# microsoft/tf-gnn-samples

Measured on AMD Instinct MI355X. Metric: edges/sec (whole node), RGCN PPI h=256 training, distinct batches (the reference's epoch-loop definition), higher is better.
Workload: dtype f32; 1 GPU; C2: RGCN on synthetic PPI-shaped batches (~16 graphs, ~1.88 M edges, ~32 k nodes each), 3 edge types [fwd,self,bkwd], h=256, 3 layers, sum aggregation, 1/in-de…; graphs_per_rank=64, max_nodes_in_batch=35964, input_pipeline=ResidentDataset, parallelism=dp1-by-graph

## Files before the change

### tf_gnn_samples_amd/csrc/seg_reduce.hip

```cpp
#include "common.h"

#include <stdlib.h>

using namespace relgnn;

namespace {

constexpr int kUnroll = 8;

__device__ __forceinline__ float act_apply(int act, float x) {
  switch (act) {
    case RELGNN_ACT_TANH: return act_fwd<RELGNN_ACT_TANH>(x);
    case RELGNN_ACT_RELU: return act_fwd<RELGNN_ACT_RELU>(x);
    case RELGNN_ACT_LEAKY_RELU: return act_fwd<RELGNN_ACT_LEAKY_RELU>(x);
    case RELGNN_ACT_ELU: return act_fwd<RELGNN_ACT_ELU>(x);
    case RELGNN_ACT_SELU: return act_fwd<RELGNN_ACT_SELU>(x);
    case RELGNN_ACT_GELU: return act_fwd<RELGNN_ACT_GELU>(x);
    default: return x;
  }
}

__device__ __forceinline__ float msg_act_apply(int act, float x) {
  switch (act) {
    case RELGNN_ACT_TANH: return act_fwd_fast<RELGNN_ACT_TANH>(x);
    case RELGNN_ACT_RELU: return act_fwd_fast<RELGNN_ACT_RELU>(x);
    case RELGNN_ACT_LEAKY_RELU: return act_fwd_fast<RELGNN_ACT_LEAKY_RELU>(x);
    case RELGNN_ACT_ELU: return act_fwd_fast<RELGNN_ACT_ELU>(x);
    case RELGNN_ACT_SELU: return act_fwd_fast<RELGNN_ACT_SELU>(x);
    case RELGNN_ACT_GELU: return act_fwd_fast<RELGNN_ACT_GELU>(x);
    default: return x;
  }
}

__device__ __forceinline__ uint32_t wave_max_u32(uint32_t v) {
  v = max(v, (uint32_t)__builtin_amdgcn_update_dpp(0, (int)v, 0xB1, 0xF, 0xF, true));
  v = max(v, (uint32_t)__builtin_amdgcn_update_dpp(0, (int)v, 0x4E, 0xF, 0xF, true));
  v = max(v, (uint32_t)__builtin_amdgcn_update_dpp(0, (int)v, 0x141, 0xF, 0xF, true));
  v = max(v, (uint32_t)__builtin_amdgcn_update_dpp(0, (int)v, 0x140, 0xF, 0xF, true));
  v = max(v, (uint32_t)__builtin_amdgcn_update_dpp(0, (int)v, 0x142, 0xA, 0xF, true));
  v = max(v, (uint32_t)__builtin_amdgcn_update_dpp(0, (int)v, 0x143, 0xC, 0xF, true));
  return (uint32_t)__builtin_amdgcn_readlane((int)v, 63);
}

template <bool IS_MAX, bool MSGACT = false>
__device__ __forceinline__ void combine(float4& acc, float w, const float4& v, int msg_act = RELGNN_ACT_LINEAR) {
  float4 m = make_float4(w * v.x, w * v.y, w * v.z, w * v.w);
  if constexpr (MSGACT) {
    m.x = msg_act_apply(msg_act, m.x); m.y = msg_act_apply(msg_act, m.y);
    m.z = msg_act_apply(msg_act, m.z); m.w = msg_act_apply(msg_act, m.w);
  }
  if constexpr (IS_MAX) {
    acc.x = fmaxf(acc.x, m.x); acc.y = fmaxf(acc.y, m.y);
    acc.z = fmaxf(acc.z, m.z); acc.w = fmaxf(acc.w, m.w);
  } else {
    acc.x += m.x; acc.y += m.y; acc.z += m.z; acc.w += m.w;
  }
}

__device__ __forceinline__ void combine64(double (&acc)[4], float w, const float4& v) {
  const double wd = (double)w;
  acc[0] = fma(wd, (double)v.x, acc[0]); acc[1] = fma(wd, (double)v.y, acc[1]);
  acc[2] = fma(wd, (double)v.z, acc[2]); acc[3] = fma(wd, (double)v.w, acc[3]);
}

__device__ __forceinline__ float4 finalize(int mode, int act, float4 a, int n) {
  if (mode == RELGNN_AGG_MEAN) {
    float d = (float)max(n, 1);
    a.x /= d; a.y /= d; a.z /= d; a.w /= d;
  } else if (mode == RELGNN_AGG_SQRT_N) {
    float d = sqrtf((float)max(n, 1));
    a.x /= d; a.y /= d; a.z /= d; a.w /= d;
  }
  if (act != RELGNN_ACT_LINEAR) {
    a.x = act_apply(act, a.x); a.y = act_apply(act, a.y);
    a.z = act_apply(act, a.z); a.w = act_apply(act, a.w);
  }
  return a;
}

template <int NCH, bool IS_MAX, bool HAS_W, int UNROLL = kUnroll, bool NT = false, bool XCD = true, bool MSGACT = false,
          bool ACC64 = false>
__global__ __launch_bounds__(256) void seg_reduce_wave_kernel(
    const float4* __restrict__ X, int64_t ldx4, int32_t D4, const int32_t* __restrict__ rowptr,
    int64_t num_segments, int32_t stride, const int32_t* __restrict__ col,
    const float* __restrict__ w, int32_t mode, int32_t act, float4* __restrict__ out, int64_t ldo4,
    int64_t n_logical_blocks, int32_t col_block0, int32_t msg_act, float* __restrict__ rowmax) {
  const int64_t lb = XCD ? xcd_logical_block(n_logical_blocks)
                         : ((int64_t)blockIdx.x < n_logical_blocks ? (int64_t)blockIdx.x : -1);
  if (lb < 0) return;
  const int lane = threadIdx.x & 63;
  const int64_t s = lb * 4 + (threadIdx.x >> 6);
  if (s >= num_segments) return;

  const int beg = __builtin_amdgcn_readfirstlane(rowptr[s * stride]);
  const int end = __builtin_amdgcn_readfirstlane(rowptr[(s + 1) * stride]);

  const int c0 = (col_block0 + (int)blockIdx.y * NCH) * 64 + lane;
  static_assert(!ACC64 || (!IS_MAX && !MSGACT), "float64 accumulation: plain sums only");
  float4 acc[NCH];
  double accd[ACC64 ? NCH : 1][4];
  bool on[NCH];
  uint32_t cc[NCH];
#pragma unroll
  for (int c = 0; c < NCH; ++c) {
    const float init = IS_MAX ? -FLT_MAX : 0.f;
    acc[c] = make_float4(init, init, init, init);
    if constexpr (ACC64) accd[c][0] = accd[c][1] = accd[c][2] = accd[c][3] = 0.0;
    on[c] = (c0 + 64 * c) < D4;
    cc[c] = (uint32_t)min(c0 + 64 * c, D4 - 1);
  }
  const uint32_t ld = (uint32_t)ldx4;

  for (int p = beg; p < end; p += 64) {
    const int n = min(64, end - p);
    const int my_col = (lane < n) ? (NT ? __builtin_nontemporal_load(col + p + lane) : col[p + lane]) : 0;
    float my_w = 1.f;
    if constexpr (HAS_W) my_w = (lane < n) ? (NT ? __builtin_nontemporal_load(w + p + lane) : w[p + lane]) : 0.f;

    int k = 0;
    for (; k + UNROLL <= n; k += UNROLL) {
      float4 v[UNROLL][NCH];
      float ww[UNROLL];
#pragma unroll
      for (int u = 0; u < UNROLL; ++u) {
        const uint32_t r = (uint32_t)__builtin_amdgcn_readlane(my_col, k + u);
        ww[u] = HAS_W ? __int_as_float(__builtin_amdgcn_readlane(__float_as_int(my_w), k + u)) : 1.f;
        const float4* row = X + (size_t)(r * ld);
#pragma unroll
        for (int c = 0; c < NCH; ++c) v[u][c] = row[cc[c]];
      }
#pragma unroll
      for (int u = 0; u < UNROLL; ++u)
#pragma unroll
        for (int c = 0; c < NCH; ++c) {
          if constexpr (ACC64) combine64(accd[c], ww[u], v[u][c]);
          else combine<IS_MAX, MSGACT>(acc[c], ww[u], v[u][c], msg_act);
        }
    }
    for (; k < n; ++k) {
      const uint32_t r = (uint32_t)__builtin_amdgcn_readlane(my_col, k);
      const float wk = HAS_W ? __int_as_float(__builtin_amdgcn_readlane(__float_as_int(my_w), k)) : 1.f;
      const float4* row = X + (size_t)(r * ld);
#pragma unroll
      for (int c = 0; c < NCH; ++c) {
        float4 v = row[cc[c]];
        if constexpr (ACC64) combine64(accd[c], wk, v);
        else combine<IS_MAX, MSGACT>(acc[c], wk, v, msg_act);
      }
    }
  }
  if constexpr (ACC64) {
#pragma unroll
    for (int c = 0; c < NCH; ++c)
      acc[c] = make_float4((float)accd[c][0], (float)accd[c][1], (float)accd[c][2], (float)accd[c][3]);
  }

  float4* orow = out + s * ldo4 + c0;
  uint32_t mxb = 0u, mxf = 0u;
  auto absb = [](float x) { return __float_as_uint(x) & 0x7FFFFFFFu; };
  auto finb = [](float x) { const uint32_t u = __float_as_uint(x) & 0x7FFFFFFFu; return u < 0x7F800000u ? u : 0u; };
#pragma unroll
  for (int c = 0; c < NCH; ++c)
    if (on[c]) {
      const float4 r = finalize(mode, act, acc[c], end - beg);
      mxb = max(max(mxb, max(absb(r.x), absb(r.y))), max(absb(r.z), absb(r.w)));
      if (__builtin_expect(mxb >= 0x7F800000u, 0))
        mxf = max(max(mxf, max(finb(r.x), finb(r.y))), max(finb(r.z), finb(r.w)));
      else
        mxf = mxb;
      if constexpr (NT) {
        float* o = reinterpret_cast<float*>(orow + 64 * c);
        __builtin_nontemporal_store(r.x, o); __builtin_nontemporal_store(r.y, o + 1);
        __builtin_nontemporal_store(r.z, o + 2); __builtin_nontemporal_store(r.w, o + 3);
      } else {
        orow[64 * c] = r;
      }
    }
  if (rowmax) {
    const uint32_t m = wave_max_u32(mxf);
    if (lane == 0) rowmax[s] = __uint_as_float(m);
  }
}

template <int GROUP, bool IS_MAX, bool HAS_W, bool MSGACT = false>
__global__ __launch_bounds__(256) void seg_reduce_group_kernel(
    const float4* __restrict__ X, int64_t ldx4, int32_t D4, const int32_t* __restrict__ rowptr,
    int64_t num_segments, int32_t stride, const int32_t* __restrict__ col,
    const float* __restrict__ w, int32_t mode, int32_t act, float4* __restrict__ out, int64_t ldo4,
    int64_t n_logical_blocks, int32_t msg_act) {
  constexpr int SEGS_PER_WAVE = 64 / GROUP;
  constexpr int U = 4;
  const int64_t lb = xcd_logical_block(n_logical_blocks);
  if (lb < 0) return;
  const int lane = threadIdx.x & 63;
  const int g = lane / GROUP, gl = lane % GROUP;
  const int64_t s = (lb * 4 + (threadIdx.x >> 6)) * SEGS_PER_WAVE + g;
  const bool valid = s < num_segments;
  const int beg = valid ? rowptr[s * stride] : 0;
  const int end = valid ? rowptr[(s + 1) * stride] : 0;
  const int len = end - beg;
  int maxlen = len;
#pragma unroll
  for (int off = 32; off >= GROUP; off >>= 1) maxlen = max(maxlen, __shfl_xor(maxlen, off));
  maxlen = __builtin_amdgcn_readfirstlane(maxlen);

  const bool on = gl < D4;
  const float init = IS_MAX ? -FLT_MAX : 0.f;
  float4 acc = make_float4(init, init, init, init);
  const float4* Xl = X + min(gl, D4 - 1);
  const uint32_t ld = (uint32_t)ldx4;

  for (int p0 = 0; p0 < maxlen; p0 += GROUP) {
    const int idx = p0 + gl;
    const int my_col = (idx < len) ? col[beg + idx] : 0;
    float my_w = 1.f;
    if constexpr (HAS_W) my_w = (idx < len) ? w[beg + idx] : 0.f;
    const int nn = min(GROUP, maxlen - p0);
    for (int k = 0; k < nn; k += U) {
      float4 v[U];
      float ww[U];
#pragma unroll
      for (int u = 0; u < U; ++u) {
        const uint32_t r = (uint32_t)__shfl(my_col, (k + u) & (GROUP - 1), GROUP);
        ww[u] = HAS_W ? __shfl(my_w, (k + u) & (GROUP - 1), GROUP) : 1.f;
        v[u] = Xl[(size_t)(r * ld)];
      }
#pragma unroll
      for (int u = 0; u < U; ++u) {
        float4 t = acc;
        combine<IS_MAX, MSGACT>(t, ww[u], v[u], msg_act);
        if (p0 + k + u < len) acc = t;
      }
    }
  }
  if (valid && on) out[s * ldo4 + gl] = finalize(mode, act, acc, len);
}

template <bool IS_MAX>
__global__ __launch_bounds__(256) void seg_reduce_scalar_kernel(
    const float* __restrict__ X, int64_t ldx, int32_t D, const int32_t* __restrict__ rowptr,
    int64_t num_segments, int32_t stride, const int32_t* __restrict__ col,
    const float* __restrict__ w, int32_t mode, int32_t act, float* __restrict__ out, int64_t ldo, int32_t msg_act) {
  const int lane = threadIdx.x & 63;
  const int64_t s = (int64_t)blockIdx.x * 4 + (threadIdx.x >> 6);
  if (s >= num_segments) return;
  const int beg = rowptr[s * stride], end = rowptr[(s + 1) * stride];
  for (int d = lane; d < D; d += 64) {
    float acc = IS_MAX ? -FLT_MAX : 0.f;
    for (int p = beg; p < end; ++p) {
      float m = msg_act_apply(msg_act, (w ? w[p] : 1.f) * X[(int64_t)col[p] * ldx + d]);
      acc = IS_MAX ? fmaxf(acc, m) : acc + m;
    }
    float nrm = (float)max(end - beg, 1);
    if (mode == RELGNN_AGG_MEAN) acc /= nrm;
    if (mode == RELGNN_AGG_SQRT_N) acc /= sqrtf(nrm);
    out[s * ldo + d] = act_apply(act, acc);
  }
}

__global__ __launch_bounds__(256) void seg_max_count_kernel(
    const float* __restrict__ X, int64_t ldx, int32_t D, const int32_t* __restrict__ rowptr,
    int64_t num_segments, int32_t stride, const int32_t* __restrict__ col,
    const float* __restrict__ w, const float* __restrict__ out, const float* __restrict__ gout,
    int64_t ldo, float* __restrict__ gsel) {
  const int lane = threadIdx.x & 63;
  const int64_t s = (int64_t)blockIdx.x * 4 + (threadIdx.x >> 6);
  if (s >= num_segments) return;
  const int beg = rowptr[s * stride], end = rowptr[(s + 1) * stride];
  for (int d = lane; d < D; d += 64) {
    const float o = out[s * ldo + d];
    float cnt = 0.f;
    for (int p = beg; p < end; ++p) {
      float m = (w ? w[p] : 1.f) * X[(int64_t)col[p] * ldx + d];
      cnt += (m == o) ? 1.f : 0.f;
    }
    gsel[s * ldo + d] = cnt > 0.f ? gout[s * ldo + d] / cnt : 0.f;
  }
}

__global__ __launch_bounds__(256) void seg_max_bwd_kernel(
    const float* __restrict__ X, int64_t ldx, int32_t D, const int32_t* __restrict__ rowptr_b,
    int64_t num_rows, int32_t stride_b, const int32_t* __restrict__ seg_b,
    const float* __restrict__ w_b, const float* __restrict__ out, const float* __restrict__ gsel,
    int64_t ldo, float* __restrict__ gX, int64_t ldgx) {
  const int lane = threadIdx.x & 63;
  const int64_t r = (int64_t)blockIdx.x * 4 + (threadIdx.x >> 6);
  if (r >= num_rows) return;
  const int beg = rowptr_b[r * stride_b], end = rowptr_b[(r + 1) * stride_b];
  for (int d = lane; d < D; d += 64) {
    const float x = X[r * ldx + d];
    float acc = 0.f;
    for (int q = beg; q < end; ++q) {
      const float wq = w_b ? w_b[q] : 1.f;
      const int64_t s = seg_b[q];
      if (wq * x == out[s * ldo + d]) acc += wq * gsel[s * ldo + d];
    }
    gX[r * ldgx + d] = acc;
  }
}

__device__ __forceinline__ float4 eq4(float4 a, float4 b) {
  return make_float4(a.x == b.x ? 1.f : 0.f, a.y == b.y ? 1.f : 0.f, a.z == b.z ? 1.f : 0.f, a.w == b.w ? 1.f : 0.f);
}

template <int G>
__global__ __launch_bounds__(256) void seg_max_count_vec_kernel(
    const float4* __restrict__ X, int64_t ldx4, int32_t D4, const int32_t* __restrict__ rowptr, int64_t num_segments,
    int32_t stride, const int32_t* __restrict__ col, const float* __restrict__ w, const float4* __restrict__ out,
    const float4* __restrict__ gout, int64_t ldo4, float4* __restrict__ gsel, int64_t nlb) {
  constexpr int U = 4;
  const int64_t lb = xcd_logical_block(nlb);
  if (lb < 0) return;
  const int lane = threadIdx.x & 63, g = lane / G, gl = lane % G;
  const int64_t s = (lb * 4 + (threadIdx.x >> 6)) * (64 / G) + g;
  if (s >= num_segments) return;
  const int beg = rowptr[s * stride], end = rowptr[(s + 1) * stride];
  for (int c = gl; c < D4; c += G) {
    const float4 o = out[s * ldo4 + c];
    float4 cnt = make_float4(0.f, 0.f, 0.f, 0.f);
    for (int p = beg; p < end; p += U) {
      int r[U];
      float ww[U];
      float4 v[U];
#pragma unroll
      for (int u = 0; u < U; ++u) {
        const int idx = min(p + u, end - 1);
        r[u] = col[idx];
        ww[u] = w ? w[idx] : 1.f;
      }
#pragma unroll
      for (int u = 0; u < U; ++u) v[u] = X[(int64_t)r[u] * ldx4 + c];
#pragma unroll
      for (int u = 0; u < U; ++u)
        if (p + u < end) {
          const float4 e = eq4(make_float4(ww[u] * v[u].x, ww[u] * v[u].y, ww[u] * v[u].z, ww[u] * v[u].w), o);
          cnt.x += e.x; cnt.y += e.y; cnt.z += e.z; cnt.w += e.w;
        }
    }
    const float4 gg = gout[s * ldo4 + c];
    gsel[s * ldo4 + c] = make_float4(cnt.x > 0.f ? gg.x / cnt.x : 0.f, cnt.y > 0.f ? gg.y / cnt.y : 0.f,
                                     cnt.z > 0.f ? gg.z / cnt.z : 0.f, cnt.w > 0.f ? gg.w / cnt.w : 0.f);
  }
}

template <int G>
__global__ __launch_bounds__(256) void seg_max_bwd_vec_kernel(
    const float4* __restrict__ X, int64_t ldx4, int32_t D4, const int32_t* __restrict__ rowptr_b, int64_t num_rows,
    int32_t stride_b, const int32_t* __restrict__ seg_b, const float* __restrict__ w_b, const float4* __restrict__ out,
    const float4* __restrict__ gsel, int64_t ldo4, float4* __restrict__ gX, int64_t ldgx4, int64_t nlb) {
  constexpr int U = 4;
  const int64_t lb = xcd_logical_block(nlb);
  if (lb < 0) return;
  const int lane = threadIdx.x & 63, g = lane / G, gl = lane % G;
  const int64_t r = (lb * 4 + (threadIdx.x >> 6)) * (64 / G) + g;
  if (r >= num_rows) return;
  const int beg = rowptr_b[r * stride_b], end = rowptr_b[(r + 1) * stride_b];
  for (int c = gl; c < D4; c += G) {
    const float4 x = X[r * ldx4 + c];
    float4 acc = make_float4(0.f, 0.f, 0.f, 0.f);
    for (int q = beg; q < end; q += U) {
      int sg[U];
      float wq[U];
      float4 o[U], gs[U];
#pragma unroll
      for (int u = 0; u < U; ++u) {
        const int idx = min(q + u, end - 1);
        sg[u] = seg_b[idx];
        wq[u] = w_b ? w_b[idx] : 1.f;
      }
#pragma unroll
      for (int u = 0; u < U; ++u) {
        o[u] = out[(int64_t)sg[u] * ldo4 + c];
        gs[u] = gsel[(int64_t)sg[u] * ldo4 + c];
      }
#pragma unroll
      for (int u = 0; u < U; ++u)
        if (q + u < end) {
          const float4 e = eq4(make_float4(wq[u] * x.x, wq[u] * x.y, wq[u] * x.z, wq[u] * x.w), o[u]);
          acc.x += e.x != 0.f ? wq[u] * gs[u].x : 0.f; acc.y += e.y != 0.f ? wq[u] * gs[u].y : 0.f;
          acc.z += e.z != 0.f ? wq[u] * gs[u].z : 0.f; acc.w += e.w != 0.f ? wq[u] * gs[u].w : 0.f;
        }
    }
    gX[r * ldgx4 + c] = acc;
  }
}

template <int ACT>
__global__ __launch_bounds__(256) void act_bwd_from_output_kernel(const float* __restrict__ y,
                                                                  const float* __restrict__ gout,
                                                                  int64_t n, float* __restrict__ gin) {
  for (int64_t i = blockIdx.x * (int64_t)blockDim.x + threadIdx.x; i < n;
       i += (int64_t)gridDim.x * blockDim.x) {
    const float yy = y[i], g = gout[i];
    float d = 1.f;
    if constexpr (ACT == RELGNN_ACT_TANH) d = 1.f - yy * yy;
    if constexpr (ACT == RELGNN_ACT_RELU) d = yy > 0.f ? 1.f : 0.f;
    if constexpr (ACT == RELGNN_ACT_LEAKY_RELU) d = yy > 0.f ? 1.f : 0.2f;
    if constexpr (ACT == RELGNN_ACT_ELU) d = yy > 0.f ? 1.f : yy + 1.f;
    if constexpr (ACT == RELGNN_ACT_SELU) {
      const float scale = 1.0507009873554804934193349852946f;
      const float scale_alpha = 1.7580993408473768599402175208123f;
      d = yy > 0.f ? scale : yy + scale_alpha;
    }
    gin[i] = g * d;
  }
}

inline int seg_variant() {
  static int v = -1;
  if (v < 0) {
    const char* e = getenv("RELGNN_SEG_VARIANT");
    v = e ? atoi(e) : 0;
  }
  return v;
}

__global__ __launch_bounds__(256) void msg_act_bwd_kernel(int32_t act, const float4* __restrict__ X, int32_t D4,
                                                          const float* __restrict__ w, const int32_t* __restrict__ tgt,
                                                          const float4* __restrict__ gagg, int64_t M,
                                                          float4* __restrict__ gX) {
  const int64_t total = M * D4;
  for (int64_t i = blockIdx.x * (int64_t)blockDim.x + threadIdx.x; i < total; i += (int64_t)gridDim.x * blockDim.x) {
    const int64_t m = i / D4;
    const int c = (int)(i - m * D4);
    const float wm = w ? w[m] : 1.f;
    const float4 x = X[i];
    const float4 g = gagg[(int64_t)tgt[m] * D4 + c];
    float4 r;
    switch (act) {
#define RELGNN_CASE(A)                                                                                             \
  case A:                                                                                                         \
    r = make_float4(wm * act_grad_fast<A>(wm * x.x) * g.x, wm * act_grad_fast<A>(wm * x.y) * g.y,                   \
                    wm * act_grad_fast<A>(wm * x.z) * g.z, wm * act_grad_fast<A>(wm * x.w) * g.w);              \
    break;
      RELGNN_CASE(RELGNN_ACT_TANH) RELGNN_CASE(RELGNN_ACT_RELU) RELGNN_CASE(RELGNN_ACT_LEAKY_RELU)
      RELGNN_CASE(RELGNN_ACT_ELU) RELGNN_CASE(RELGNN_ACT_SELU) RELGNN_CASE(RELGNN_ACT_GELU)
#undef RELGNN_CASE
      default: r = make_float4(wm * g.x, wm * g.y, wm * g.z, wm * g.w); break;
    }
    gX[i] = r;
  }
}

thread_local float* tl_rowmax = nullptr;

template <int NCH, bool IS_MAX>
int launch_wave(bool has_w, const float* X, int64_t ldx, int32_t D, const int32_t* rowptr,
                int64_t S, int32_t stride, const int32_t* col, const float* w, int32_t mode,
                int32_t act, float* out, int64_t ldo, hipStream_t st, int32_t msg_act, bool acc64 = false) {
  const int D4 = D / 4;
  const int64_t nlb = (S + 3) / 4;
  const int col_blocks = (D4 + 64 * NCH - 1) / (64 * NCH);
  dim3 grid((unsigned)(((nlb + 7) / 8) * 8), (unsigned)col_blocks);
  if constexpr (!IS_MAX) {
    if (acc64) {
      if (msg_act != RELGNN_ACT_LINEAR) return RELGNN_EUNSUPPORTED;
      if (has_w)
        seg_reduce_wave_kernel<NCH, false, true, kUnroll, false, true, false, true><<<grid, 256, 0, st>>>(
            reinterpret_cast<const float4*>(X), ldx / 4, D4, rowptr, S, stride, col, w, mode, act,
            reinterpret_cast<float4*>(out), ldo / 4, nlb, 0, msg_act, tl_rowmax);
      else
        seg_reduce_wave_kernel<NCH, false, false, kUnroll, false, true, false, true><<<grid, 256, 0, st>>>(
            reinterpret_cast<const float4*>(X), ldx / 4, D4, rowptr, S, stride, col, w, mode, act,
            reinterpret_cast<float4*>(out), ldo / 4, nlb, 0, msg_act, tl_rowmax);
      return launch_status();
    }
  }
  if constexpr (NCH == 1 && !IS_MAX) {
    const int var = seg_variant();
    if (var != 0 && has_w) {
#define RELGNN_VARIANT_CASE(ID, U, N, X_)                                                              \
  case ID:                                                                                             \
    seg_reduce_wave_kernel<1, false, true, U, N, X_><<<grid, 256, 0, st>>>(                            \
        reinterpret_cast<const float4*>(X), ldx / 4, D4, rowptr, S, stride, col, w, mode, act,         \
        reinterpret_cast<float4*>(out), ldo / 4, nlb, 0, msg_act, tl_rowmax);                                     \
    return launch_status();
      switch (var) {
        RELGNN_VARIANT_CASE(1, 16, false, true)
        RELGNN_VARIANT_CASE(2, 8, true, true)
        RELGNN_VARIANT_CASE(3, 16, true, true)
        RELGNN_VARIANT_CASE(4, 8, false, false)
        RELGNN_VARIANT_CASE(5, 16, false, false)
        RELGNN_VARIANT_CASE(6, 8, true, false)
        RELGNN_VARIANT_CASE(7, 16, true, false)
        RELGNN_VARIANT_CASE(8, 4, false, true)
        default: break;
      }
#undef RELGNN_VARIANT_CASE
    }
  }
  if (msg_act != RELGNN_ACT_LINEAR) {
    if (has_w)
      seg_reduce_wave_kernel<NCH, IS_MAX, true, kUnroll, false, true, true><<<grid, 256, 0, st>>>(
          reinterpret_cast<const float4*>(X), ldx / 4, D4, rowptr, S, stride, col, w, mode, act,
          reinterpret_cast<float4*>(out), ldo / 4, nlb, 0, msg_act, tl_rowmax);
    else
      seg_reduce_wave_kernel<NCH, IS_MAX, false, kUnroll, false, true, true><<<grid, 256, 0, st>>>(
          reinterpret_cast<const float4*>(X), ldx / 4, D4, rowptr, S, stride, col, w, mode, act,
          reinterpret_cast<float4*>(out), ldo / 4, nlb, 0, msg_act, tl_rowmax);
    return launch_status();
  }
  if (has_w)
    seg_reduce_wave_kernel<NCH, IS_MAX, true><<<grid, 256, 0, st>>>(
        reinterpret_cast<const float4*>(X), ldx / 4, D4, rowptr, S, stride, col, w, mode, act,
        reinterpret_cast<float4*>(out), ldo / 4, nlb, 0, msg_act, tl_rowmax);
  else
    seg_reduce_wave_kernel<NCH, IS_MAX, false><<<grid, 256, 0, st>>>(
        reinterpret_cast<const float4*>(X), ldx / 4, D4, rowptr, S, stride, col, w, mode, act,
        reinterpret_cast<float4*>(out), ldo / 4, nlb, 0, msg_act, tl_rowmax);
  return launch_status();
}

template <int GROUP, bool IS_MAX>
int launch_group(bool has_w, const float* X, int64_t ldx, int32_t D, const int32_t* rowptr,
                 int64_t S, int32_t stride, const int32_t* col, const float* w, int32_t mode,
                 int32_t act, float* out, int64_t ldo, hipStream_t st, int32_t msg_act) {
  constexpr int SEGS_PER_BLOCK = 4 * (64 / GROUP);
  const int64_t nlb = (S + SEGS_PER_BLOCK - 1) / SEGS_PER_BLOCK;
  dim3 grid((unsigned)(((nlb + 7) / 8) * 8));
  if (msg_act != RELGNN_ACT_LINEAR) {
    if (has_w)
      seg_reduce_group_kernel<GROUP, IS_MAX, true, true><<<grid, 256, 0, st>>>(
          reinterpret_cast<const float4*>(X), ldx / 4, D / 4, rowptr, S, stride, col, w, mode, act,
          reinterpret_cast<float4*>(out), ldo / 4, nlb, msg_act);
    else
      seg_reduce_group_kernel<GROUP, IS_MAX, false, true><<<grid, 256, 0, st>>>(
          reinterpret_cast<const float4*>(X), ldx / 4, D / 4, rowptr, S, stride, col, w, mode, act,
          reinterpret_cast<float4*>(out), ldo / 4, nlb, msg_act);
    return launch_status();
  }
  if (has_w)
    seg_reduce_group_kernel<GROUP, IS_MAX, true><<<grid, 256, 0, st>>>(
        reinterpret_cast<const float4*>(X), ldx / 4, D / 4, rowptr, S, stride, col, w, mode, act,
        reinterpret_cast<float4*>(out), ldo / 4, nlb, msg_act);
  else
    seg_reduce_group_kernel<GROUP, IS_MAX, false><<<grid, 256, 0, st>>>(
        reinterpret_cast<const float4*>(X), ldx / 4, D / 4, rowptr, S, stride, col, w, mode, act,
        reinterpret_cast<float4*>(out), ldo / 4, nlb, msg_act);
  return launch_status();
}

template <bool IS_MAX>
int dispatch_fwd(const float* X, int64_t num_rows_x, int64_t ldx, int32_t D, const int32_t* rowptr, int64_t S,
                 int32_t stride, const int32_t* col, const float* w, int32_t mode, int32_t act,
                 float* out, int64_t ldo, hipStream_t st, int32_t msg_act, bool acc64 = false) {
  const bool vec_ok = (D % 4 == 0) && (ldx % 4 == 0) && (ldo % 4 == 0) && aligned16(X) &&
                      aligned16(out) && (num_rows_x * (ldx / 4) < ((int64_t)1 << 32));
  if (acc64) {
    if (IS_MAX || !vec_ok || D / 4 <= 32 || D / 4 > 256) return RELGNN_EUNSUPPORTED;
    const bool has_w = w != nullptr;
    if (D / 4 <= 64) return launch_wave<1, IS_MAX>(has_w, X, ldx, D, rowptr, S, stride, col, w, mode, act, out, ldo, st, msg_act, true);
    if (D / 4 <= 128) return launch_wave<2, IS_MAX>(has_w, X, ldx, D, rowptr, S, stride, col, w, mode, act, out, ldo, st, msg_act, true);
    return launch_wave<4, IS_MAX>(has_w, X, ldx, D, rowptr, S, stride, col, w, mode, act, out, ldo, st, msg_act, true);
  }
  if (!vec_ok) {
    seg_reduce_scalar_kernel<IS_MAX><<<(unsigned)((S + 3) / 4), 256, 0, st>>>(
        X, ldx, D, rowptr, S, stride, col, w, mode, act, out, ldo, msg_act);
    return launch_status();
  }
  const bool has_w = w != nullptr;
  const int D4 = D / 4;
  if (D4 <= 8) return launch_group<8, IS_MAX>(has_w, X, ldx, D, rowptr, S, stride, col, w, mode, act, out, ldo, st, msg_act);
  if (D4 <= 16) return launch_group<16, IS_MAX>(has_w, X, ldx, D, rowptr, S, stride, col, w, mode, act, out, ldo, st, msg_act);
  if (D4 <= 32) return launch_group<32, IS_MAX>(has_w, X, ldx, D, rowptr, S, stride, col, w, mode, act, out, ldo, st, msg_act);
  if (D4 <= 64) return launch_wave<1, IS_MAX>(has_w, X, ldx, D, rowptr, S, stride, col, w, mode, act, out, ldo, st, msg_act);
  if (D4 <= 128) return launch_wave<2, IS_MAX>(has_w, X, ldx, D, rowptr, S, stride, col, w, mode, act, out, ldo, st, msg_act);
  return launch_wave<4, IS_MAX>(has_w, X, ldx, D, rowptr, S, stride, col, w, mode, act, out, ldo, st, msg_act);
}

}

extern "C" {

static int seg_reduce_any(int32_t mode, int32_t msg_act, const float* X, int64_t num_rows_x, int64_t ldx, int32_t D,
                          const int32_t* rowptr, int64_t num_segments, int32_t seg_stride, const int32_t* col,
                          const float* w, int32_t act, float* out, int64_t ldo, void* stream, bool acc64 = false);

int relgnn_seg_reduce_acc64_fwd(int32_t mode, const float* X, int64_t num_rows_x, int64_t ldx, int32_t D,
                                const int32_t* rowptr, int64_t num_segments, int32_t seg_stride,
                                const int32_t* col, const float* w, int32_t act, float* out, int64_t ldo,
                                void* stream) {
  if (mode == RELGNN_AGG_MAX) return RELGNN_EINVAL;
  return seg_reduce_any(mode, RELGNN_ACT_LINEAR, X, num_rows_x, ldx, D, rowptr, num_segments, seg_stride, col, w, act,
                        out, ldo, stream, true);
}

int relgnn_seg_reduce_fwd(int32_t mode, const float* X, int64_t num_rows_x, int64_t ldx, int32_t D,
                          const int32_t* rowptr, int64_t num_segments, int32_t seg_stride,
                          const int32_t* col, const float* w, int32_t act, float* out, int64_t ldo,
                          void* stream) {
  return seg_reduce_any(mode, RELGNN_ACT_LINEAR, X, num_rows_x, ldx, D, rowptr, num_segments, seg_stride, col, w, act,
                        out, ldo, stream);
}

int relgnn_seg_reduce_fwd_rowmax(int32_t mode, const float* X, int64_t num_rows_x, int64_t ldx, int32_t D,
                                 const int32_t* rowptr, int64_t num_segments, int32_t seg_stride,
                                 const int32_t* col, const float* w, int32_t act, float* out, int64_t ldo,
                                 float* rowmax, void* stream) {
  if (!rowmax) return RELGNN_EINVAL;
  if (mode == RELGNN_AGG_MAX || D % 4 != 0 || D <= 128 || D > 1024 || ldx % 4 != 0 || ldo % 4 != 0 || !aligned16(X) || !aligned16(out) ||
      num_rows_x * (ldx / 4) >= ((int64_t)1 << 32))
    return RELGNN_EUNSUPPORTED;
  tl_rowmax = rowmax;
  const int rc = seg_reduce_any(mode, RELGNN_ACT_LINEAR, X, num_rows_x, ldx, D, rowptr, num_segments, seg_stride, col, w, act,
                                out, ldo, stream);
  tl_rowmax = nullptr;
  return rc;
}

int relgnn_seg_reduce_msgact_fwd(int32_t mode, int32_t msg_act, const float* X, int64_t num_rows_x, int64_t ldx,
                                 int32_t D, const int32_t* rowptr, int64_t num_segments, int32_t seg_stride,
                                 const int32_t* col, const float* w, float* out, int64_t ldo, void* stream) {
  if (msg_act < RELGNN_ACT_LINEAR || msg_act > RELGNN_ACT_GELU) return RELGNN_EINVAL;
  return seg_reduce_any(mode, msg_act, X, num_rows_x, ldx, D, rowptr, num_segments, seg_stride, col, w,
                        RELGNN_ACT_LINEAR, out, ldo, stream);
}

static int seg_reduce_any(int32_t mode, int32_t msg_act, const float* X, int64_t num_rows_x, int64_t ldx, int32_t D,
                          const int32_t* rowptr, int64_t num_segments, int32_t seg_stride, const int32_t* col,
                          const float* w, int32_t act, float* out, int64_t ldo, void* stream, bool acc64) {
  if (mode < RELGNN_AGG_SUM || mode > RELGNN_AGG_MAX) return RELGNN_EINVAL;
  if (act < RELGNN_ACT_LINEAR || act > RELGNN_ACT_GELU) return RELGNN_EINVAL;
  if (D < 0 || num_segments < 0 || seg_stride <= 0 || num_rows_x < 0 || ldx < D || ldo < D)
    return RELGNN_EINVAL;
  if (num_segments == 0 || D == 0) return RELGNN_OK;
  if (!rowptr || !out) return RELGNN_EINVAL;
  if (num_segments > (int64_t)INT32_MAX * 4) return RELGNN_EUNSUPPORTED;
  hipStream_t st = as_stream(stream);
  if (mode == RELGNN_AGG_MAX)
    return dispatch_fwd<true>(X, num_rows_x, ldx, D, rowptr, num_segments, seg_stride, col, w, mode, act, out, ldo, st, msg_act);
  return dispatch_fwd<false>(X, num_rows_x, ldx, D, rowptr, num_segments, seg_stride, col, w, mode, act, out, ldo, st, msg_act,
                             acc64);
}

int relgnn_msg_act_bwd(int32_t act, const float* X, int32_t D, const float* w, const int32_t* tgt, const float* gagg,
                       int64_t num_messages, float* gX, void* stream) {
  if (act < RELGNN_ACT_LINEAR || act > RELGNN_ACT_GELU || D < 0 || num_messages < 0) return RELGNN_EINVAL;
  if (num_messages == 0 || D == 0) return RELGNN_OK;
  if (!X || !tgt || !gagg || !gX) return RELGNN_EINVAL;
  if (D % 4 != 0 || !aligned16(X) || !aligned16(gagg) || !aligned16(gX)) return RELGNN_EUNSUPPORTED;
  msg_act_bwd_kernel<<<flat_grid(num_messages * (D / 4), 256), 256, 0, as_stream(stream)>>>(
      act, (const float4*)X, D / 4, w, tgt, (const float4*)gagg, num_messages, (float4*)gX);
  return launch_status();
}

int relgnn_seg_max_count(const float* X, int64_t ldx, int32_t D, const int32_t* rowptr,
                         int64_t num_segments, int32_t seg_stride, const int32_t* col,
                         const float* w, const float* out, const float* gout, int64_t ldo,
                         float* gsel, void* stream) {
  if (D < 0 || num_segments < 0 || seg_stride <= 0) return RELGNN_EINVAL;
  if (num_segments == 0 || D == 0) return RELGNN_OK;
  if (!rowptr || !out || !gout || !gsel) return RELGNN_EINVAL;
  if (D % 4 == 0 && ldx % 4 == 0 && ldo % 4 == 0 && aligned16(X) && aligned16(out) && aligned16(gout) && aligned16(gsel)) {
    const int D4 = D / 4;
    hipStream_t st = as_stream(stream);
#define RELGNN_MAXCNT(GG)                                                                                              \
  {                                                                                                                    \
    const int64_t nlb = (num_segments + 4 * (64 / GG) - 1) / (4 * (64 / GG));                                          \
    seg_max_count_vec_kernel<GG><<<(unsigned)(((nlb + 7) / 8) * 8), 256, 0, st>>>(                                      \
        (const float4*)X, ldx / 4, D4, rowptr, num_segments, seg_stride, col, w, (const float4*)out, (const float4*)gout, \
        ldo / 4, (float4*)gsel, nlb);                                                                                  \
  }
    if (D4 <= 8) RELGNN_MAXCNT(8) else if (D4 <= 16) RELGNN_MAXCNT(16) else if (D4 <= 32) RELGNN_MAXCNT(32) else RELGNN_MAXCNT(64)
#undef RELGNN_MAXCNT
    return launch_status();
  }
  seg_max_count_kernel<<<(unsigned)((num_segments + 3) / 4), 256, 0, as_stream(stream)>>>(
      X, ldx, D, rowptr, num_segments, seg_stride, col, w, out, gout, ldo, gsel);
  return launch_status();
}

int relgnn_seg_max_bwd(const float* X, int64_t ldx, int32_t D, const int32_t* rowptr_b,
                       int64_t num_rows_x, int32_t seg_stride_b, const int32_t* seg_b,
                       const float* w_b, const float* out, const float* gsel, int64_t ldo,
                       float* gX, int64_t ldgx, void* stream) {
  if (D < 0 || num_rows_x < 0 || seg_stride_b <= 0) return RELGNN_EINVAL;
  if (num_rows_x == 0 || D == 0) return RELGNN_OK;
  if (!X || !rowptr_b || !gX) return RELGNN_EINVAL;
  if (D % 4 == 0 && ldx % 4 == 0 && ldo % 4 == 0 && ldgx % 4 == 0 && aligned16(X) && aligned16(out) && aligned16(gsel) &&
      aligned16(gX)) {
    const int D4 = D / 4;
    hipStream_t st = as_stream(stream);
#define RELGNN_MAXBWD(GG)                                                                                              \
  {                                                                                                                    \
    const int64_t nlb = (num_rows_x + 4 * (64 / GG) - 1) / (4 * (64 / GG));                                            \
    seg_max_bwd_vec_kernel<GG><<<(unsigned)(((nlb + 7) / 8) * 8), 256, 0, st>>>(                                        \
        (const float4*)X, ldx / 4, D4, rowptr_b, num_rows_x, seg_stride_b, seg_b, w_b, (const float4*)out,              \
        (const float4*)gsel, ldo / 4, (float4*)gX, ldgx / 4, nlb);                                                     \
  }
    if (D4 <= 8) RELGNN_MAXBWD(8) else if (D4 <= 16) RELGNN_MAXBWD(16) else if (D4 <= 32) RELGNN_MAXBWD(32) else RELGNN_MAXBWD(64)
#undef RELGNN_MAXBWD
    return launch_status();
  }
  seg_max_bwd_kernel<<<(unsigned)((num_rows_x + 3) / 4), 256, 0, as_stream(stream)>>>(
      X, ldx, D, rowptr_b, num_rows_x, seg_stride_b, seg_b, w_b, out, gsel, ldo, gX, ldgx);
  return launch_status();
}

int relgnn_act_bwd_from_output(int32_t act, const float* y, const float* gout, int64_t n, float* gin,
                               void* stream) {
  if (n < 0) return RELGNN_EINVAL;
  if (act == RELGNN_ACT_GELU) return RELGNN_EUNSUPPORTED;
  if (n == 0) return RELGNN_OK;
  if (!y || !gout || !gin) return RELGNN_EINVAL;
  hipStream_t st = as_stream(stream);
  RELGNN_DISPATCH_ACT(act, A,
                      (act_bwd_from_output_kernel<A><<<flat_grid(n, 256), 256, 0, st>>>(y, gout, n, gin)));
  return launch_status();
}

}
```

Measured before the change: 1.028 billion edges/sec.

## Add block-cooperative path for long segments and prefetch edge indices in seg_reduce

Factors the per-wave segment reduction into a helper. The helper prefetches the next chunk of column indices while the current one is processed, handles the tail with a compile-time dispatch instead of a scalar loop, and uses byte offsets for row loads. For NCH==1 plain-sum kernels, segments with 64 or more edges are handed to a cooperative path: all four waves of the block split the feature columns and process four edges per step through an LDS transpose. The change also adds an occupancy hint and optional timing instrumentation. The trade-off is extra __syncthreads and LDS traffic in every COOP kernel, plus register-pressure risk from the waves-per-eu attribute.

```diff
diff --git a/tf_gnn_samples_amd/csrc/seg_reduce.hip b/tf_gnn_samples_amd/csrc/seg_reduce.hip
--- a/tf_gnn_samples_amd/csrc/seg_reduce.hip
+++ b/tf_gnn_samples_amd/csrc/seg_reduce.hip
@@ -2,11 +2,17 @@
 
 #include <stdlib.h>
 
+#include <type_traits>
+
 using namespace relgnn;
 
 namespace {
 
 constexpr int kUnroll = 8;
+
+#ifdef RELGNN_SEG_TIMING
+__device__ unsigned long long* g_seg_timing_dev = nullptr;
+#endif
 
 __device__ __forceinline__ float act_apply(int act, float x) {
   switch (act) {
@@ -78,29 +84,26 @@
   return a;
 }
 
-template <int NCH, bool IS_MAX, bool HAS_W, int UNROLL = kUnroll, bool NT = false, bool XCD = true, bool MSGACT = false,
-          bool ACC64 = false>
-__global__ __launch_bounds__(256) void seg_reduce_wave_kernel(
-    const float4* __restrict__ X, int64_t ldx4, int32_t D4, const int32_t* __restrict__ rowptr,
-    int64_t num_segments, int32_t stride, const int32_t* __restrict__ col,
-    const float* __restrict__ w, int32_t mode, int32_t act, float4* __restrict__ out, int64_t ldo4,
-    int64_t n_logical_blocks, int32_t col_block0, int32_t msg_act, float* __restrict__ rowmax) {
-  const int64_t lb = XCD ? xcd_logical_block(n_logical_blocks)
-                         : ((int64_t)blockIdx.x < n_logical_blocks ? (int64_t)blockIdx.x : -1);
-  if (lb < 0) return;
-  const int lane = threadIdx.x & 63;
-  const int64_t s = lb * 4 + (threadIdx.x >> 6);
-  if (s >= num_segments) return;
-
-  const int beg = __builtin_amdgcn_readfirstlane(rowptr[s * stride]);
-  const int end = __builtin_amdgcn_readfirstlane(rowptr[(s + 1) * stride]);
-
+template <int N, class F>
+__device__ __forceinline__ void dispatch_below(int r, F&& f) {
+  if constexpr (N > 0) {
+    if (r == N - 1) f(std::integral_constant<int, N - 1>{});
+    else dispatch_below<N - 1>(r, f);
+  }
+}
+
+template <int NCH, bool IS_MAX, bool HAS_W, int UNROLL, bool NT, bool MSGACT, bool ACC64>
+__device__ __forceinline__ void seg_wave_fold(
+    const float4* __restrict__ X, int64_t ldx4, int32_t D4, const int32_t* __restrict__ col, const float* __restrict__ w,
+    int32_t mode, int32_t act, float4* __restrict__ out, int64_t ldo4, int32_t col_block0, int32_t msg_act,
+    float* __restrict__ rowmax, int64_t s, int lane, int beg, int end) {
   const int c0 = (col_block0 + (int)blockIdx.y * NCH) * 64 + lane;
   static_assert(!ACC64 || (!IS_MAX && !MSGACT), "float64 accumulation: plain sums only");
   float4 acc[NCH];
   double accd[ACC64 ? NCH : 1][4];
   bool on[NCH];
   uint32_t cc[NCH];
+  uint32_t cb[NCH];
 #pragma unroll
   for (int c = 0; c < NCH; ++c) {
     const float init = IS_MAX ? -FLT_MAX : 0.f;
@@ -108,46 +111,69 @@
     if constexpr (ACC64) accd[c][0] = accd[c][1] = accd[c][2] = accd[c][3] = 0.0;
     on[c] = (c0 + 64 * c) < D4;
     cc[c] = (uint32_t)min(c0 + 64 * c, D4 - 1);
+    cb[c] = cc[c] * 16u;
   }
   const uint32_t ld = (uint32_t)ldx4;
 
+  static_assert(UNROLL % 4 == 0 && UNROLL >= 4, "row loads are issued in slots of four");
+  constexpr int H = 4, NS = UNROLL / H;
+  float4 v[UNROLL][NCH];
+  float ww[UNROLL];
+  int my_col = 0;
+  float my_w = 1.f;
+  auto load_index = [&](int p, int n, int& ci, float& wi) __attribute__((always_inline)) {
+    ci = (lane < n) ? (NT ? __builtin_nontemporal_load(col + p + lane) : col[p + lane]) : 0;
+    if constexpr (HAS_W) wi = (lane < n) ? (NT ? __builtin_nontemporal_load(w + p + lane) : w[p + lane]) : 0.f;
+  };
+  auto issue = [&](int u, int k) __attribute__((always_inline)) {
+    const uint32_t r = (uint32_t)__builtin_amdgcn_readlane(my_col, k);
+    ww[u] = HAS_W ? __int_as_float(__builtin_amdgcn_readlane(__float_as_int(my_w), k)) : 1.f;
+    const char* row = reinterpret_cast<const char*>(X + (size_t)(r * ld));
+#pragma unroll
+    for (int c = 0; c < NCH; ++c) v[u][c] = *reinterpret_cast<const float4*>(row + cb[c]);
+  };
+  auto fold = [&](int u) __attribute__((always_inline)) {
+#pragma unroll
+    for (int c = 0; c < NCH; ++c) {
+      if constexpr (ACC64) combine64(accd[c], ww[u], v[u][c]);
+      else combine<IS_MAX, MSGACT>(acc[c], ww[u], v[u][c], msg_act);
+    }
+  };
+  auto slot_issue = [&](int j, int k, int cnt) __attribute__((always_inline)) {
+#pragma unroll
+    for (int u = 0; u < H; ++u)
+      if (u < cnt) issue(j * H + u, k + u);
+  };
+  auto slot_fold = [&](int j, int cnt) __attribute__((always_inline)) {
+#pragma unroll
+    for (int u = 0; u < H; ++u)
+      if (u < cnt) fold(j * H + u);
+  };
+  auto tail = [&](auto r_c, int k) __attribute__((always_inline)) {
+    constexpr int R = decltype(r_c)::value;
+#pragma unroll
+    for (int j = 0; j < NS; ++j) slot_issue(j, k + H * j, R - H * j);
+#pragma unroll
+    for (int j = 0; j < NS; ++j) slot_fold(j, R - H * j);
+  };
+
+  if (beg < end) load_index(beg, min(64, end - beg), my_col, my_w);
   for (int p = beg; p < end; p += 64) {
     const int n = min(64, end - p);
-    const int my_col = (lane < n) ? (NT ? __builtin_nontemporal_load(col + p + lane) : col[p + lane]) : 0;
-    float my_w = 1.f;
-    if constexpr (HAS_W) my_w = (lane < n) ? (NT ? __builtin_nontemporal_load(w + p + lane) : w[p + lane]) : 0.f;
+    int nx_col = 0;
+    float nx_w = 1.f;
+    if (p + 64 < end) load_index(p + 64, min(64, end - p - 64), nx_col, nx_w);
 
     int k = 0;
     for (; k + UNROLL <= n; k += UNROLL) {
-      float4 v[UNROLL][NCH];
-      float ww[UNROLL];
-#pragma unroll
-      for (int u = 0; u < UNROLL; ++u) {
-        const uint32_t r = (uint32_t)__builtin_amdgcn_readlane(my_col, k + u);
-        ww[u] = HAS_W ? __int_as_float(__builtin_amdgcn_readlane(__float_as_int(my_w), k + u)) : 1.f;
-        const float4* row = X + (size_t)(r * ld);
-#pragma unroll
-        for (int c = 0; c < NCH; ++c) v[u][c] = row[cc[c]];
-      }
-#pragma unroll
-      for (int u = 0; u < UNROLL; ++u)
-#pragma unroll
-        for (int c = 0; c < NCH; ++c) {
-          if constexpr (ACC64) combine64(accd[c], ww[u], v[u][c]);
-          else combine<IS_MAX, MSGACT>(acc[c], ww[u], v[u][c], msg_act);
-        }
-    }
-    for (; k < n; ++k) {
-      const uint32_t r = (uint32_t)__builtin_amdgcn_readlane(my_col, k);
-      const float wk = HAS_W ? __int_as_float(__builtin_amdgcn_readlane(__float_as_int(my_w), k)) : 1.f;
-      const float4* row = X + (size_t)(r * ld);
-#pragma unroll
-      for (int c = 0; c < NCH; ++c) {
-        float4 v = row[cc[c]];
-        if constexpr (ACC64) combine64(accd[c], wk, v);
-        else combine<IS_MAX, MSGACT>(acc[c], wk, v, msg_act);
-      }
-    }
+#pragma unroll
+      for (int j = 0; j < NS; ++j) slot_issue(j, k + H * j, H);
+#pragma unroll
+      for (int j = 0; j < NS; ++j) slot_fold(j, H);
+    }
+    if (k < n) dispatch_below<UNROLL>(n - k, [&](auto r_c) __attribute__((always_inline)) { tail(r_c, k); });
+    my_col = nx_col;
+    my_w = nx_w;
   }
   if constexpr (ACC64) {
 #pragma unroll
@@ -180,6 +206,122 @@
     const uint32_t m = wave_max_u32(mxf);
     if (lane == 0) rowmax[s] = __uint_as_float(m);
   }
+}
+
+constexpr int kCoopMin = 64;
+
+constexpr int kCoopWords = 17 * 15 + 4 * 3 + 3 + 1;
+
+template <bool HAS_W>
+__device__ __forceinline__ void seg_coop_fold(
+    const float4* __restrict__ X, int64_t ldx4, int32_t D4, const int32_t* __restrict__ rowptr, int32_t stride,
+    const int32_t* __restrict__ col, const float* __restrict__ w, int32_t mode, int32_t act, float4* __restrict__ out,
+    int64_t ldo4, float* __restrict__ rowmax, int64_t s, int wv, int lane, float* turn, uint32_t* s_max) {
+  const int beg = __builtin_amdgcn_readfirstlane(rowptr[s * stride]);
+  const int end = __builtin_amdgcn_readfirstlane(rowptr[(s + 1) * stride]);
+  const int q = lane >> 4, i = lane & 15;
+  const int c = wv * 16 + i;
+  const int f = 4 * i + q;
+  const char* Xc = reinterpret_cast<const char*>(X) + (size_t)min(c, D4 - 1) * 16;
+  const uint32_t ld = (uint32_t)ldx4;
+  float* put = turn + 17 * i + q;
+  const float* get = turn + 17 * (f >> 2) + 4 * (f & 3);
+  float acc = 0.f;
+  for (int p = beg; p < end; p += 64) {
+    const int n = min(64, end - p);
+    const int my_col = (lane < n) ? col[p + lane] : 0;
+    float my_w = 1.f;
+    if constexpr (HAS_W) my_w = (lane < n) ? w[p + lane] : 0.f;
+    for (int k = 0; k < n; k += 4 * kUnroll) {
+      float4 v[kUnroll];
+#pragma unroll
+      for (int u = 0; u < kUnroll; ++u) {
+        const int mi = min(k + 4 * u + q, n - 1);
+        const uint32_t r = (uint32_t)__builtin_amdgcn_ds_bpermute(mi * 4, my_col);
+        v[u] = *reinterpret_cast<const float4*>(Xc + (size_t)(r * ld) * 16);
+      }
+#pragma unroll
+      for (int u = 0; u < kUnroll; ++u) {
+        const int mi = min(k + 4 * u + q, n - 1);
+        const float wq = HAS_W ? __int_as_float(__builtin_amdgcn_ds_bpermute(mi * 4, __float_as_int(my_w))) : 1.f;
+        __builtin_amdgcn_fence(__ATOMIC_ACQ_REL, "wavefront");
+        put[0] = wq * v[u].x; put[4] = wq * v[u].y; put[8] = wq * v[u].z; put[12] = wq * v[u].w;
+        __builtin_amdgcn_fence(__ATOMIC_ACQ_REL, "wavefront");
+        const float m0 = get[0], m1 = get[1], m2 = get[2], m3 = get[3];
+        __builtin_amdgcn_fence(__ATOMIC_ACQ_REL, "wavefront");
+        const int left = n - (k + 4 * u);
+        if (left > 0) acc += m0;
+        if (left > 1) acc += m1;
+        if (left > 2) acc += m2;
+        if (left > 3) acc += m3;
+      }
+    }
+  }
+  const int cnt = end - beg;
+  if (mode == RELGNN_AGG_MEAN) acc /= (float)max(cnt, 1);
+  else if (mode == RELGNN_AGG_SQRT_N) acc /= sqrtf((float)max(cnt, 1));
+  if (act != RELGNN_ACT_LINEAR) acc = act_apply(act, acc);
+  const bool writer = 64 * wv + f < 4 * D4;
+  if (writer) reinterpret_cast<float*>(out + s * ldo4)[64 * wv + f] = acc;
+  if (rowmax) {
+    const uint32_t ab = __float_as_uint(acc) & 0x7FFFFFFFu;
+    const uint32_t m = wave_max_u32(writer && ab < 0x7F800000u ? ab : 0u);
+    if (lane == 0) s_max[wv] = m;
+    __syncthreads();
+    if (threadIdx.x == 0) rowmax[s] = __uint_as_float(max(max(s_max[0], s_max[1]), max(s_max[2], s_max[3])));
+    __syncthreads();
+  }
+}
+
+template <int NCH, bool IS_MAX, bool HAS_W, int UNROLL = kUnroll, bool NT = false, bool XCD = true, bool MSGACT = false,
+          bool ACC64 = false>
+__global__ __launch_bounds__(256)
+__attribute__((amdgpu_waves_per_eu((NCH == 1 && !ACC64 && !MSGACT && UNROLL <= 8) ? 8 : 1))) void seg_reduce_wave_kernel(
+    const float4* __restrict__ X, int64_t ldx4, int32_t D4, const int32_t* __restrict__ rowptr,
+    int64_t num_segments, int32_t stride, const int32_t* __restrict__ col,
+    const float* __restrict__ w, int32_t mode, int32_t act, float4* __restrict__ out, int64_t ldo4,
+    int64_t n_logical_blocks, int32_t col_block0, int32_t msg_act, float* __restrict__ rowmax) {
+  const int64_t lb = XCD ? xcd_logical_block(n_logical_blocks)
+                         : ((int64_t)blockIdx.x < n_logical_blocks ? (int64_t)blockIdx.x : -1);
+  if (lb < 0) return;
+  const int lane = threadIdx.x & 63, wv = threadIdx.x >> 6;
+  const int64_t s = lb * 4 + wv;
+#ifdef RELGNN_SEG_TIMING
+  const unsigned long long ts0 = __builtin_amdgcn_s_memtime();
+#endif
+  constexpr bool COOP = NCH == 1 && !IS_MAX && !MSGACT && !ACC64 && !NT;
+  __shared__ uint32_t s_long[4], s_max[4];
+  __shared__ float s_turn[COOP ? 4 * kCoopWords : 1];
+  const bool valid = s < num_segments;
+  const int beg = valid ? __builtin_amdgcn_readfirstlane(rowptr[s * stride]) : 0;
+  const int end = valid ? __builtin_amdgcn_readfirstlane(rowptr[(s + 1) * stride]) : 0;
+  bool is_long = false;
+  if constexpr (COOP) {
+    is_long = valid && end - beg >= kCoopMin && D4 <= 64 && gridDim.y == 1;
+    if (lane == 0) s_long[wv] = is_long ? 1u : 0u;
+  }
+  if (valid && !is_long)
+    seg_wave_fold<NCH, IS_MAX, HAS_W, UNROLL, NT, MSGACT, ACC64>(X, ldx4, D4, col, w, mode, act, out, ldo4, col_block0, msg_act,
+                                                                  rowmax, s, lane, beg, end);
+  if constexpr (COOP) {
+    __syncthreads();
+#pragma unroll 1
+    for (int j = 0; j < 4; ++j)
+      if (__builtin_amdgcn_readfirstlane((int)s_long[j]))
+        seg_coop_fold<HAS_W>(X, ldx4, D4, rowptr, stride, col, w, mode, act, out, ldo4, rowmax, lb * 4 + j, wv, lane,
+                             s_turn + (COOP ? wv * kCoopWords : 0), s_max);
+  }
+#ifdef RELGNN_SEG_TIMING
+  {
+    __builtin_amdgcn_sched_barrier(0);
+    const unsigned long long ts1 = __builtin_amdgcn_s_memtime();
+    unsigned long long* t = g_seg_timing_dev;
+    if (t && valid && lane == 0 && blockIdx.y == 0) {
+      t[4 * s + 0] = ts0; t[4 * s + 1] = ts1;
+      t[4 * s + 2] = (unsigned long long)(end - beg); t[4 * s + 3] = blockIdx.x;
+    }
+  }
+#endif
 }
 
 template <int GROUP, bool IS_MAX, bool HAS_W, bool MSGACT = false>
@@ -585,6 +727,12 @@
                         out, ldo, stream, true);
 }
 
+#ifdef RELGNN_SEG_TIMING
+int relgnn_seg_timing_buffer(void* buf) {
+  return hipMemcpyToSymbol(HIP_SYMBOL(g_seg_timing_dev), &buf, sizeof(buf)) == hipSuccess ? RELGNN_OK : RELGNN_EINVAL;
+}
+#endif
+
 int relgnn_seg_reduce_fwd(int32_t mode, const float* X, int64_t num_rows_x, int64_t ldx, int32_t D,
                           const int32_t* rowptr, int64_t num_segments, int32_t seg_stride,
                           const int32_t* col, const float* w, int32_t act, float* out, int64_t ldo,
```

Result: slower. 1.002 billion edges/sec (-2.5%).
